# play-with-HOI-generation/HOIG

Hardware: AMD Instinct MI355X
Metric: HOGAN train images/sec at 256x256 (higher is better)
Workload: dtype f16x3 fwd (both operands split hi+lo on fp16, 3 MFMAs per product) / bf16x2 bwd (dy split hi+lo, weights and x single bf16, 2 MFMAs per product), f32 accumulate; 1 GPU; 256x256 HO3Dv3-shaped synthetic, batch 8 per GPU, G+D full step (generator_spade_attn, VGG19 surrogate weights); global_batch=8, parallelism=dp1

## Files before the change

hoig_amd/csrc/common.h:

```cpp
#pragma once
#include <hip/hip_runtime.h>
#include <stdint.h>
#include <atomic>
#include "hoig_kernels.h"

typedef float f32x16 __attribute__((ext_vector_type(16)));
typedef float f32x4 __attribute__((ext_vector_type(4)));
typedef short bf16x8 __attribute__((ext_vector_type(8)));

#define HOIG_LAUNCH_CHECK()                                   \
    do {                                                      \
        hipError_t e__ = hipGetLastError();                   \
        if (e__ != hipSuccess) return HOIG_ELAUNCH;           \
    } while (0)

struct hoig_once {
    std::atomic<unsigned long long> mask{0};
    static int dev() {
        int d = 0;
        (void)hipGetDevice(&d);
        return d & 63;
    }
    bool done() const { return (mask.load(std::memory_order_acquire) >> dev()) & 1ull; }
    void set() { mask.fetch_or(1ull << dev(), std::memory_order_release); }
};

static inline int64_t hoig_cdiv(int64_t a, int64_t b) { return (a + b - 1) / b; }

int hoig_conv_small_fwd(const hoig_conv_desc *d, const float *x, const float *w, const float *bias, float *y, hipStream_t st);
int hoig_conv_small_fwd_acts(const hoig_conv_desc *d, const float *x, const float *w, const float *bias, float *y,
                             unsigned long long acts, hipStream_t st);
int hoig_conv_small_ci_fwd(const hoig_conv_desc *d, const float *x, const float *w, const float *bias, float *y, hipStream_t st);
int hoig_conv_small_dgrad(const hoig_conv_desc *d, const float *dy, const float *w, float *dx, hipStream_t st);
int hoig_conv_small_wgrad(const hoig_conv_desc *d, const float *x, const float *dy, float *dw, hipStream_t st);
int hoig_conv_dot_fwd(const hoig_conv_desc *d, const float *x, const float *w, const float *bias, float *y, hipStream_t st);
int hoig_conv_head7_m16(const hoig_conv_desc *d, const float *x, const float *w, const float *bias, float *y, unsigned long long acts,
                        hipStream_t st);
int hoig_conv_thin_fwd(const hoig_conv_desc *d, const float *x, const float *w, const float *bias, float *y, hipStream_t st,
                       double *stats = nullptr);
int hoig_conv_thin_dgrad(const hoig_conv_desc *d, const float *dy, const float *w, float *dx, int accumulate, hipStream_t st);
int hoig_conv_thin_wgrad(const hoig_conv_desc *d, const float *x, const float *dy, float *dw, hipStream_t st);
bool hoig_conv_thin_wgrad_applies(const hoig_conv_desc *d);
int hoig_conv_thin_out(const hoig_conv_desc *d, const float *x, const float *w, const float *bias, float *y, unsigned long long acts,
                       int dgrad, hipStream_t st);
int hoig_conv_bf16_wgrad(const hoig_conv_desc *d, const float *x, const float *dy, float *dw, float *dbias, hipStream_t st);
bool hoig_conv_bf16_wgrad_fuses_bias(const hoig_conv_desc *d);
namespace hoig_detail { void *stream_scratch(hipStream_t st, size_t bytes); }

static inline int hoig_stream_grid(int64_t work_items, int block) {
    int64_t g = hoig_cdiv(work_items, block);
    if (g > 2048) g = 2048;
    if (g < 1) g = 1;
    return (int)g;
}

__device__ __forceinline__ float hoig_act(float v, int act, float slope) {
    switch (act) {
        case HOIG_ACT_RELU: return v > 0.f ? v : 0.f;
        case HOIG_ACT_LRELU: return v > 0.f ? v : v * slope;
        case HOIG_ACT_TANH: return tanhf(v);
        case HOIG_ACT_SIGMOID: return 1.f / (1.f + expf(-v));
        default: return v;
    }
}

__device__ __forceinline__ float fast_act(float v, float nslope, bool special, int act, float slope) {
    if (special) return hoig_act(v, act, slope);
    return v > 0.f ? v : fmaf(v, nslope, 0.f);
}

__device__ __forceinline__ float hoig_act_grad_from_y(float y, int act, float slope) {
    switch (act) {
        case HOIG_ACT_RELU: return y > 0.f ? 1.f : 0.f;
        case HOIG_ACT_LRELU: return y > 0.f ? 1.f : slope;
        case HOIG_ACT_TANH: return 1.f - y * y;
        case HOIG_ACT_SIGMOID: return y * (1.f - y);
        default: return 1.f;
    }
}

__device__ __forceinline__ void hoig_stats_add(double *stats, int b, int N, int mom, int n, float v) {
    atomicAdd(stats + ((size_t)b * 2 + mom) * N + n, (double)v);
}

__device__ __forceinline__ int hoig_xcd_remap(int bid, int nblk) {
    const int q = nblk >> 3, r = nblk & 7, xcd = bid & 7, idx = bid >> 3;
    const int base = xcd < r ? xcd * (q + 1) : r * (q + 1) + (xcd - r) * q;
    return base + idx;
}

__device__ __forceinline__ float hoig_wave_sum(float v) {
#pragma unroll
    for (int o = 32; o > 0; o >>= 1) v += __shfl_xor(v, o, 64);
    return v;
}

__device__ __forceinline__ unsigned short hoig_f2bf(float f) {
    unsigned int u = __float_as_uint(f);
    u += 0x7FFFu + ((u >> 16) & 1u);
    return (unsigned short)(u >> 16);
}
__device__ __forceinline__ float hoig_bf2f(unsigned short h) { return __uint_as_float(((unsigned int)h) << 16); }
```

hoig_amd/csrc/conv_thin.hip:

```cpp
#include "common.h"
#include <map>
#include <mutex>

namespace {

typedef _Float16 f16x8 __attribute__((ext_vector_type(8)));
typedef short s16x4 __attribute__((ext_vector_type(4)));

constexpr int TH = 4, TW = 32, NTHR = 256;

struct ThinArgs {
    const float *T;
    const float *D;
    const float *bias;
    float *Out;
    float *Ws;
    int Bn, H, W, F, CD, KS, pad;
    int flip;
    int sj, st, sf;
    int act;
    float slope;
    int accumulate;
    float wscale;
    int K, KP, N, NP;
    int tiles_x, tiles_y, ntiles, strip;
    int HR, CW;
    double *stats;
};

template <bool FP16>
__device__ __forceinline__ void split16(float x, unsigned short &hi, unsigned short &lo) {
    if (FP16) {
        const _Float16 h = (_Float16)x;
        const _Float16 l = (_Float16)(x - (float)h);
        hi = __builtin_bit_cast(unsigned short, h);
        lo = __builtin_bit_cast(unsigned short, l);
    } else {
        const __bf16 h = (__bf16)x;
        hi = __builtin_bit_cast(unsigned short, h);
        const __bf16 l = (__bf16)(x - hoig_bf2f(hi));
        lo = __builtin_bit_cast(unsigned short, l);
    }
}

template <bool FP16>
__device__ __forceinline__ f32x16 mfma16(const bf16x8 a, const bf16x8 b, const f32x16 c) {
    if (FP16) return __builtin_amdgcn_mfma_f32_32x32x16_f16(__builtin_bit_cast(f16x8, a), __builtin_bit_cast(f16x8, b), c, 0, 0, 0);
    return __builtin_amdgcn_mfma_f32_32x32x16_bf16(a, b, c, 0, 0, 0);
}

constexpr int HMAX = 12;
struct HaloRegs {
    float v[HMAX];
};
struct HaloMap {
    int lds[HMAX];
    int rc[HMAX];
    int rounds;
};
__device__ __forceinline__ void halo_map(const ThinArgs &p, HaloMap &m) {
    const int wr = TW + p.KS - 1;
    const int row_elems = wr * p.F;
    const int total = p.HR * row_elems;
    m.rounds = (total + NTHR - 1) / NTHR;
#pragma unroll
    for (int it = 0; it < HMAX; ++it) {
        const int i = threadIdx.x + it * NTHR;
        m.lds[it] = -1;
        m.rc[it] = 0;
        if (i < total) {
            const int hy = i / row_elems, e = i - hy * row_elems;
            const int hx = e / p.F, f = e - hx * p.F;
            m.lds[it] = (f * p.HR + hy) * p.CW + hx;
            m.rc[it] = hy | (hx << 8) | (f << 16);
        }
    }
}
__device__ __forceinline__ void halo_load(const ThinArgs &p, const HaloMap &m, int b, int y0, int x0, HaloRegs &h) {
    const float *img = p.T + (size_t)b * p.H * p.W * p.F;
#pragma unroll
    for (int it = 0; it < HMAX; ++it) {
        h.v[it] = 0.f;
        if (it < m.rounds && m.lds[it] >= 0) {
            const int gy = y0 - p.pad + (m.rc[it] & 255), gx = x0 - p.pad + ((m.rc[it] >> 8) & 255);
            if (gy >= 0 && gy < p.H && gx >= 0 && gx < p.W) h.v[it] = img[((size_t)gy * p.W + gx) * p.F + (m.rc[it] >> 16)];
        }
    }
}
template <bool FP16, int NT>
__device__ __forceinline__ void halo_store(const ThinArgs &p, const HaloMap &m, const HaloRegs &h, unsigned short *Tl) {
    const int plane = p.F * p.HR * p.CW;
#pragma unroll
    for (int it = 0; it < HMAX; ++it)
        if (it < m.rounds && m.lds[it] >= 0) {
            unsigned short hi, lo;
            split16<FP16>(h.v[it], hi, lo);
            Tl[m.lds[it]] = hi;
            if (NT == 2) Tl[plane + m.lds[it]] = lo;
        }
}

__device__ __forceinline__ void tile_coords(const ThinArgs &p, int t, int &b, int &y0, int &x0) {
    const int tx = t % p.tiles_x;
    t /= p.tiles_x;
    const int ty = t % p.tiles_y;
    b = t / p.tiles_y;
    y0 = ty * TH;
    x0 = tx * TW;
}

template <bool FP16, int NT, int NW>
__global__ __launch_bounds__(NTHR) void thin_gemm_kernel(const ThinArgs p) {
    extern __shared__ __attribute__((aligned(16))) unsigned char smem[];
    const int wstride = p.KP + 8;
    unsigned short *Wl = reinterpret_cast<unsigned short *>(smem);
    unsigned short *toff = Wl + NW * 64 * wstride;
    unsigned short *Tl = toff + p.KP;
    const int tid = threadIdx.x, lane = tid & 63, wave = tid >> 6;
    const int l31 = lane & 31, lh = lane >> 5;
    const int cbase = blockIdx.y * 64;
    const int KK = p.KS * p.KS;
    const int tplane = p.F * p.HR * p.CW;

    for (int i0 = tid; i0 < 64 * p.KP; i0 += 4 * NTHR) {
        float v[4];
        int dst[4];
#pragma unroll
        for (int u = 0; u < 4; ++u) {
            const int i = i0 + u * NTHR;
            v[u] = 0.f;
            dst[u] = -1;
            if (i < 64 * p.KP) {
                const int n = i / p.KP, k = i - n * p.KP;
                dst[u] = n * wstride + k;
                if (k < p.K) {
                    const int tap = k / p.F, f = k - tap * p.F;
                    const int tw = p.flip ? KK - 1 - tap : tap;
                    v[u] = p.D[(size_t)(cbase + n) * p.sj + (size_t)tw * p.st + (size_t)f * p.sf];
                }
            }
        }
#pragma unroll
        for (int u = 0; u < 4; ++u)
            if (dst[u] >= 0) {
                unsigned short hi, lo;
                split16<FP16>(v[u] * p.wscale, hi, lo);
                Wl[dst[u]] = hi;
                if (NW == 2) Wl[64 * wstride + dst[u]] = lo;
            }
    }
    for (int k = tid; k < p.KP; k += NTHR) {
        const int kc = k < p.K ? k : p.K - 1;
        const int tap = kc / p.F, f = kc - tap * p.F;
        const int r = tap / p.KS, s = tap - r * p.KS;
        toff[k] = (unsigned short)((f * p.HR + r) * p.CW + s);
    }

    const float nslope = p.act == HOIG_ACT_NONE ? 1.f : (p.act == HOIG_ACT_RELU ? 0.f : p.slope);
    const bool special = p.act == HOIG_ACT_TANH || p.act == HOIG_ACT_SIGMOID;
    const float inv = 1.f / p.wscale;
    float bias_r[2];
#pragma unroll
    for (int j = 0; j < 2; ++j) bias_r[j] = p.bias ? p.bias[cbase + j * 32 + l31] : 0.f;
    const int ksteps = p.KP >> 4;
    const int pix = wave * p.CW + l31;

    const int t_end = min(p.ntiles, (int)(blockIdx.x + 1) * p.strip);
    HaloRegs hreg;
    HaloMap hmap;
    halo_map(p, hmap);
    {
        int b, y0, x0;
        tile_coords(p, blockIdx.x * p.strip, b, y0, x0);
        halo_load(p, hmap, b, y0, x0, hreg);
    }
    float st1[2] = {0.f, 0.f}, st2[2] = {0.f, 0.f};
    int sb = -1;
    auto flush_stats = [&]() {
        if (sb >= 0) {
#pragma unroll
            for (int j = 0; j < 2; ++j) {
                const float s1 = st1[j] + __shfl_xor(st1[j], 32), s2 = st2[j] + __shfl_xor(st2[j], 32);
                if (lh == 0) {
                    hoig_stats_add(p.stats, sb, p.CD, 0, cbase + j * 32 + l31, s1);
                    hoig_stats_add(p.stats, sb, p.CD, 1, cbase + j * 32 + l31, s2);
                }
                st1[j] = st2[j] = 0.f;
            }
        }
    };
    for (int t = blockIdx.x * p.strip; t < t_end; ++t) {
        int b, y0, x0;
        tile_coords(p, t, b, y0, x0);
        if (p.stats && b != sb) {
            flush_stats();
            sb = b;
        }
        __syncthreads();
        halo_store<FP16, NT>(p, hmap, hreg, Tl);
        __syncthreads();
        if (t + 1 < t_end) {
            int b2, y2, x2;
            tile_coords(p, t + 1, b2, y2, x2);
            halo_load(p, hmap, b2, y2, x2, hreg);
        }
        f32x16 acc[2];
#pragma unroll
        for (int j = 0; j < 2; ++j)
#pragma unroll
            for (int r = 0; r < 16; ++r) acc[j][r] = 0.f;
#pragma unroll 1
        for (int kk = 0; kk < ksteps; ++kk) {
            const int k0 = kk * 16 + lh * 8;
            const bf16x8 offs = *reinterpret_cast<const bf16x8 *>(toff + k0);
            bf16x8 a0, a1;
#pragma unroll
            for (int e = 0; e < 8; ++e) {
                const int o = (int)(unsigned short)offs[e] + pix;
                a0[e] = (short)Tl[o];
                if (NT == 2) a1[e] = (short)Tl[tplane + o];
            }
#pragma unroll
            for (int j = 0; j < 2; ++j) {
                const unsigned short *wr = Wl + (j * 32 + l31) * wstride + k0;
                const bf16x8 w0 = *reinterpret_cast<const bf16x8 *>(wr);
                if (NT == 2) acc[j] = mfma16<FP16>(a1, w0, acc[j]);
                if (NW == 2) acc[j] = mfma16<FP16>(a0, *reinterpret_cast<const bf16x8 *>(wr + 64 * wstride), acc[j]);
                acc[j] = mfma16<FP16>(a0, w0, acc[j]);
            }
        }
        const int oy = y0 + wave;
#pragma unroll
        for (int r = 0; r < 16; ++r) {
            const int ox = x0 + (r & 3) + 8 * (r >> 2) + 4 * lh;
            float *dst = p.Out + (((size_t)b * p.H + oy) * p.W + ox) * p.CD + cbase + l31;
#pragma unroll
            for (int j = 0; j < 2; ++j) {
                float v = acc[j][r] * inv + bias_r[j];
                v = fast_act(v, nslope, special, p.act, p.slope);
                if (p.accumulate) v += dst[j * 32];
                dst[j * 32] = v;
                st1[j] += v;
                st2[j] += v * v;
            }
        }
    }
    if (p.stats) flush_stats();
}

constexpr int DROW = 192;

template <int NPW, int WN, int NT, int ND>
__global__ __launch_bounds__(NTHR) void thin_wgrad_kernel(const ThinArgs p) {
    constexpr int WK = 4 / WN, NPIX = TH * TW, KSTEPS = NPIX / 16;
    extern __shared__ __attribute__((aligned(16))) unsigned char smem[];
    unsigned char *Dl = smem;
    unsigned short *Tl = reinterpret_cast<unsigned short *>(smem + ND * NPIX * DROW);
    float *Gl = reinterpret_cast<float *>(smem);
    const int tid = threadIdx.x, lane = tid & 63, wave = tid >> 6;
    const int l31 = lane & 31, lh = lane >> 5;
    const int wn = wave % WN, wk = wave / WN;
    const int cbase = blockIdx.y * 64;
    const int KK = p.KS * p.KS;
    const int tplane = p.F * p.HR * p.CW;

    int noff[NPW];
    bool nval[NPW];
#pragma unroll
    for (int j = 0; j < NPW; ++j) {
        const int n = (wn * NPW + j) * 32 + l31;
        nval[j] = n < p.N;
        const int nc = nval[j] ? n : 0;
        const int tap = nc / p.F, f = nc - tap * p.F;
        const int tt = p.flip ? KK - 1 - tap : tap;
        const int r = tt / p.KS, s = tt - r * p.KS;
        noff[j] = (f * p.HR + r) * p.CW + s + lh * 8;
    }
    const int g = lane >> 4, q = (lane >> 2) & 3, pp = lane & 3;
    const int a_off = (8 * (g >> 1) + q) * DROW + (16 * (g & 1) + 4 * pp) * 2;

    f32x16 acc[2][NPW];
#pragma unroll
    for (int i = 0; i < 2; ++i)
#pragma unroll
        for (int j = 0; j < NPW; ++j)
#pragma unroll
            for (int r = 0; r < 16; ++r) acc[i][j][r] = 0.f;

    constexpr int DT = NPIX * 8 / NTHR;
    float4 dreg[DT][2];
    auto load_d = [&](int t) {
        int b, y0, x0;
        tile_coords(p, t, b, y0, x0);
#pragma unroll
        for (int i = 0; i < DT; ++i) {
            const int task = tid + i * NTHR, px = task >> 3, c8 = task & 7;
            const int yy = y0 + (px >> 5), xx = x0 + (px & 31);
            const float *src = p.D + (((size_t)b * p.H + yy) * p.W + xx) * p.CD + cbase + c8 * 8;
            dreg[i][0] = *reinterpret_cast<const float4 *>(src);
            dreg[i][1] = *reinterpret_cast<const float4 *>(src + 4);
        }
    };
    auto store_d = [&]() {
#pragma unroll
        for (int i = 0; i < DT; ++i) {
            const int task = tid + i * NTHR, px = task >> 3, c8 = task & 7;
            const float v[8] = {dreg[i][0].x, dreg[i][0].y, dreg[i][0].z, dreg[i][0].w,
                                dreg[i][1].x, dreg[i][1].y, dreg[i][1].z, dreg[i][1].w};
            bf16x8 hi, lo;
#pragma unroll
            for (int e = 0; e < 8; e += 2) {
                typedef float f2v __attribute__((ext_vector_type(2)));
                typedef __bf16 b2v __attribute__((ext_vector_type(2)));
                const f2v x2 = {v[e], v[e + 1]};
                const unsigned hp = __builtin_bit_cast(unsigned, __builtin_convertvector(x2, b2v));
                hi[e] = (short)(hp & 0xffffu);
                hi[e + 1] = (short)(hp >> 16);
                if (ND == 2) {
                    const f2v r2 = {v[e] - __uint_as_float(hp << 16), v[e + 1] - __uint_as_float(hp & 0xffff0000u)};
                    const unsigned lp = __builtin_bit_cast(unsigned, __builtin_convertvector(r2, b2v));
                    lo[e] = (short)(lp & 0xffffu);
                    lo[e + 1] = (short)(lp >> 16);
                }
            }
            *reinterpret_cast<bf16x8 *>(Dl + px * DROW + c8 * 16) = hi;
            if (ND == 2) *reinterpret_cast<bf16x8 *>(Dl + NPIX * DROW + px * DROW + c8 * 16) = lo;
        }
    };

    int t = blockIdx.x;
    HaloRegs hreg;
    HaloMap hmap;
    halo_map(p, hmap);
    if (t < p.ntiles) {
        int b, y0, x0;
        tile_coords(p, t, b, y0, x0);
        load_d(t);
        halo_load(p, hmap, b, y0, x0, hreg);
    }
    for (; t < p.ntiles; t += gridDim.x) {
        __syncthreads();
        store_d();
        halo_store<false, NT>(p, hmap, hreg, Tl);
        __syncthreads();
        if (t + (int)gridDim.x < p.ntiles) {
            int b, y0, x0;
            tile_coords(p, t + gridDim.x, b, y0, x0);
            load_d(t + gridDim.x);
            halo_load(p, hmap, b, y0, x0, hreg);
        }
#pragma unroll 1
        for (int ks = wk; ks < KSTEPS; ks += WK) {
            const int prow = ks >> 1, pcol = (ks & 1) * 16;
            bf16x8 a[2][ND];
#pragma unroll
            for (int i = 0; i < 2; ++i)
#pragma unroll
                for (int d = 0; d < ND; ++d) {
                    const unsigned char *src = Dl + d * NPIX * DROW + (prow * 32 + pcol) * DROW + a_off + i * 64;
                    const s16x4 v0 = __builtin_amdgcn_ds_read_tr16_b64_v4i16((__attribute__((address_space(3))) s16x4 *)(src));
                    const s16x4 v1 = __builtin_amdgcn_ds_read_tr16_b64_v4i16((__attribute__((address_space(3))) s16x4 *)(src + 4 * DROW));
                    a[i][d] = (bf16x8){v0[0], v0[1], v0[2], v0[3], v1[0], v1[1], v1[2], v1[3]};
                }
            const int base = prow * p.CW + pcol;
#pragma unroll
            for (int j = 0; j < NPW; ++j) {
                bf16x8 b0, b1;
#pragma unroll
                for (int e = 0; e < 8; ++e) {
                    const int o = base + noff[j] + e;
                    b0[e] = nval[j] ? (short)Tl[o] : (short)0;
                    if (NT == 2) b1[e] = nval[j] ? (short)Tl[tplane + o] : (short)0;
                }
#pragma unroll
                for (int i = 0; i < 2; ++i) {
                    if (ND == 2) acc[i][j] = mfma16<false>(a[i][1], b0, acc[i][j]);
                    if (NT == 2) acc[i][j] = mfma16<false>(a[i][0], b1, acc[i][j]);
                    acc[i][j] = mfma16<false>(a[i][0], b0, acc[i][j]);
                }
            }
        }
    }

    __syncthreads();
    for (int i = tid; i < 64 * p.NP; i += NTHR) Gl[i] = 0.f;
    __syncthreads();
#pragma unroll
    for (int i = 0; i < 2; ++i)
#pragma unroll
        for (int j = 0; j < NPW; ++j) {
            const int n = (wn * NPW + j) * 32 + l31;
            if (n < p.NP)
#pragma unroll
                for (int r = 0; r < 16; ++r) {
                    const int m = i * 32 + (r & 3) + 8 * (r >> 2) + 4 * lh;
                    if (WK > 1) atomicAdd(&Gl[m * p.NP + n], acc[i][j][r]);
                    else Gl[m * p.NP + n] = acc[i][j][r];
                }
        }
    __syncthreads();
    if (p.Ws) {
        float *dst = p.Ws + ((size_t)blockIdx.y * gridDim.x + blockIdx.x) * 64 * p.NP;
        for (int i = tid; i < 64 * p.NP; i += NTHR) dst[i] = Gl[i];
        return;
    }
    if (p.sj == 1) {
        for (int i = tid; i < 64 * p.N; i += NTHR) {
            const int n = i >> 6, m = i & 63;
            const int tap = n / p.F, f = n - tap * p.F;
            atomicAdd(p.Out + (size_t)f * p.sf + (size_t)tap * p.st + cbase + m, Gl[m * p.NP + n]);
        }
    } else {
        for (int i = tid; i < 64 * p.N; i += NTHR) {
            const int m = i / p.N, n = i - m * p.N;
            const int tap = n / p.F, f = n - tap * p.F;
            atomicAdd(p.Out + (size_t)(cbase + m) * p.sj + (size_t)tap * p.st + (size_t)f * p.sf, Gl[m * p.NP + n]);
        }
    }
}

__global__ __launch_bounds__(NTHR) void thin_reduce_kernel(const ThinArgs p, int nwg) {
    const int cbase = blockIdx.y * 64;
    const float *src = p.Ws + (size_t)blockIdx.y * nwg * 64 * p.NP;
    const int i = blockIdx.x * NTHR + threadIdx.x;
    if (i >= 64 * p.N) return;
    const int m = i / p.N, n = i - m * p.N;
    const int wper = (nwg + (int)gridDim.z - 1) / (int)gridDim.z;
    const int w0 = blockIdx.z * wper, w1 = min(nwg, w0 + wper);
    const size_t step = (size_t)64 * p.NP;
    const float *col = src + m * p.NP + n + (size_t)w0 * step;
    float v0 = 0.f, v1 = 0.f, v2 = 0.f, v3 = 0.f;
    int w = w0;
    for (; w + 3 < w1; w += 4, col += 4 * step) {
        v0 += col[0];
        v1 += col[step];
        v2 += col[2 * step];
        v3 += col[3 * step];
    }
    for (; w < w1; ++w, col += step) v0 += col[0];
    const float v = (v0 + v1) + (v2 + v3);
    const int tap = n / p.F, f = n - tap * p.F;
    atomicAdd(p.Out + (size_t)(cbase + m) * p.sj + (size_t)tap * p.st + (size_t)f * p.sf, v);
}

constexpr size_t WS_SLOT_BYTES = (size_t)16 << 20;
float *thin_workspace(hipStream_t st, size_t bytes) { return static_cast<float *>(hoig_detail::stream_scratch(st, bytes)); }

typedef float f32x4v __attribute__((ext_vector_type(4)));

struct ThinOutArgs {
    const float *D, *Wt, *bias;
    float *Out;
    int Bn, H, W, F, CD, KS, pad, flip;
    int sf, st, sj;
    unsigned long long acts;
    float slope, wscale;
    int tiles_x, tiles_y, ntiles, strip, HR, HWc;
};

template <bool FP16>
__device__ __forceinline__ f32x4v mfma16x16(const bf16x8 a, const bf16x8 b, const f32x4v c) {
    if (FP16) return __builtin_amdgcn_mfma_f32_16x16x32_f16(__builtin_bit_cast(f16x8, a), __builtin_bit_cast(f16x8, b), c, 0, 0, 0);
    return __builtin_amdgcn_mfma_f32_16x16x32_bf16(a, b, c, 0, 0, 0);
}

template <bool FP16, int ND, int NW>
__global__ __launch_bounds__(NTHR) void thin_out_kernel(const ThinOutArgs p) {
    constexpr int PROW = 80, WROW = 144;
    extern __shared__ __attribute__((aligned(16))) unsigned char smem[];
    const int KK = p.KS * p.KS, hpix = p.HR * p.HWc;
    unsigned char *Wl = smem;
    unsigned char *Dl = smem + (size_t)NW * (p.CD >> 6) * p.F * KK * WROW;
    const int tid = threadIdx.x, lane = tid & 63, wave = tid >> 6;
    const int l15 = lane & 15, kg = lane >> 4;
    const int wplane = p.F * KK * WROW;

    for (int i0 = tid; i0 < p.F * KK * p.CD; i0 += 4 * NTHR) {
        float v[4];
        int dst[4];
#pragma unroll
        for (int u = 0; u < 4; ++u) {
            const int i = i0 + u * NTHR;
            v[u] = 0.f;
            dst[u] = -1;
            if (i < p.F * KK * p.CD) {
                const int j = i % p.CD, ft = i / p.CD;
                const int tap = ft % KK, f = ft / KK;
                const int tw = p.flip ? KK - 1 - tap : tap;
                v[u] = p.Wt[(size_t)f * p.sf + (size_t)tw * p.st + (size_t)j * p.sj];
                dst[u] = ((j >> 6) * p.F * KK + f * KK + tap) * WROW + (j & 63) * 2;
            }
        }
#pragma unroll
        for (int u = 0; u < 4; ++u)
            if (dst[u] >= 0) {
                unsigned short hi, lo;
                split16<FP16>(v[u] * p.wscale, hi, lo);
                *reinterpret_cast<unsigned short *>(Wl + dst[u]) = hi;
                if (NW == 2) *reinterpret_cast<unsigned short *>(Wl + (size_t)(p.CD >> 6) * wplane + dst[u]) = lo;
            }
    }

    int apix[2];
#pragma unroll
    for (int i = 0; i < 2; ++i) {
        const int g = 2 * wave + i;
        apix[i] = ((g >> 1) * p.HWc + 16 * (g & 1) + l15) * PROW + kg * 16;
    }
    const bool nvalid = l15 < p.F;
    const int wrow0 = l15 * KK * WROW + kg * 16;
    const float inv = 1.f / p.wscale;
    const int act_n = (int)((p.acts >> (4 * l15)) & 15);
    const float bias_n = (p.bias && nvalid) ? p.bias[l15] : 0.f;

    constexpr int HT = 12;
    float4 hreg[HT];
    auto halo_load = [&](int t, int kh) {
        int b, y0, x0;
        const int tx = t % p.tiles_x, r1 = t / p.tiles_x;
        b = r1 / p.tiles_y;
        y0 = (r1 % p.tiles_y) * TH;
        x0 = tx * TW;
#pragma unroll
        for (int it = 0; it < HT; ++it) {
            const int i = tid + it * NTHR;
            hreg[it] = make_float4(0.f, 0.f, 0.f, 0.f);
            if (it * NTHR < hpix * 8 && i < hpix * 8) {
                const int px = i >> 3, c4 = i & 7;
                const int hy = px / p.HWc, hx = px - hy * p.HWc;
                const int gy = y0 - p.pad + hy, gx = x0 - p.pad + hx;
                if (gy >= 0 && gy < p.H && gx >= 0 && gx < p.W)
                    hreg[it] = *reinterpret_cast<const float4 *>(p.D + (((size_t)b * p.H + gy) * p.W + gx) * p.CD + kh * 32 + c4 * 4);
            }
        }
    };
    auto halo_store = [&]() {
#pragma unroll
        for (int it = 0; it < HT; ++it) {
            const int i = tid + it * NTHR;
            if (it * NTHR < hpix * 8 && i < hpix * 8) {
                const int px = i >> 3, c4 = i & 7;
                const float v[4] = {hreg[it].x, hreg[it].y, hreg[it].z, hreg[it].w};
                unsigned short h[4], l[4];
#pragma unroll
                for (int e = 0; e < 4; ++e) split16<FP16>(v[e], h[e], l[e]);
                *reinterpret_cast<uint2 *>(Dl + px * PROW + c4 * 8) = make_uint2(h[0] | ((unsigned)h[1] << 16), h[2] | ((unsigned)h[3] << 16));
                if (ND == 2)
                    *reinterpret_cast<uint2 *>(Dl + hpix * PROW + px * PROW + c4 * 8) =
                        make_uint2(l[0] | ((unsigned)l[1] << 16), l[2] | ((unsigned)l[3] << 16));
            }
        }
    };

    const int nkh = p.CD >> 5;
    const int t_begin = blockIdx.x * p.strip, t_end = min(p.ntiles, t_begin + p.strip);
    if (t_begin < t_end) halo_load(t_begin, 0);
    for (int t = t_begin; t < t_end; ++t) {
        f32x4v acc[2];
#pragma unroll
        for (int i = 0; i < 2; ++i) acc[i] = (f32x4v){0.f, 0.f, 0.f, 0.f};
        for (int kh = 0; kh < nkh; ++kh) {
            __syncthreads();
            halo_store();
            __syncthreads();
            if (kh + 1 < nkh) halo_load(t, kh + 1);
            else if (t + 1 < t_end) halo_load(t + 1, 0);
            const unsigned char *wbase = Wl + (size_t)(kh >> 1) * wplane + wrow0 + (kh & 1) * 64;
#pragma unroll 1
            for (int tap = 0; tap < KK; ++tap) {
                const int r = tap / p.KS, s_ = tap - r * p.KS;
                const int toff = (r * p.HWc + s_) * PROW;
                bf16x8 bh = {0, 0, 0, 0, 0, 0, 0, 0}, bl = bh;
                if (nvalid) {
                    bh = *reinterpret_cast<const bf16x8 *>(wbase + tap * WROW);
                    if (NW == 2) bl = *reinterpret_cast<const bf16x8 *>(wbase + (size_t)(p.CD >> 6) * wplane + tap * WROW);
                }
#pragma unroll
                for (int i = 0; i < 2; ++i) {
                    const unsigned char *ap = Dl + apix[i] + toff;
                    const bf16x8 ah = *reinterpret_cast<const bf16x8 *>(ap);
                    if (ND == 2) acc[i] = mfma16x16<FP16>(*reinterpret_cast<const bf16x8 *>(ap + hpix * PROW), bh, acc[i]);
                    if (NW == 2) acc[i] = mfma16x16<FP16>(ah, bl, acc[i]);
                    acc[i] = mfma16x16<FP16>(ah, bh, acc[i]);
                }
            }
        }
        if (nvalid) {
            const int tx = t % p.tiles_x, r1 = t / p.tiles_x;
            const int b = r1 / p.tiles_y, y0 = (r1 % p.tiles_y) * TH, x0 = tx * TW;
#pragma unroll
            for (int i = 0; i < 2; ++i) {
                const int g = 2 * wave + i;
                const int oy = y0 + (g >> 1), oxb = x0 + 16 * (g & 1) + 4 * kg;
#pragma unroll
                for (int e = 0; e < 4; ++e) {
                    const float v = acc[i][e] * inv + bias_n;
                    p.Out[(((size_t)b * p.H + oy) * p.W + oxb + e) * p.F + l15] = hoig_act(v, act_n, p.slope);
                }
            }
        }
    }
}

bool thin_geometry(const hoig_conv_desc *d) {
    return !d->transposed && d->stride == 1 && d->R == d->S && (d->R & 1) && d->R <= 7 && 2 * d->pad == d->R - 1 &&
           d->Ho == d->Hi && d->Wo == d->Wi && (d->Hi % TH) == 0 && (d->Wi % TW) == 0;
}

void fill_common(ThinArgs &a, const hoig_conv_desc *d, int F, int CD) {
    a.Bn = d->B; a.H = d->Hi; a.W = d->Wi; a.F = F; a.CD = CD; a.KS = d->R; a.pad = d->pad;
    a.K = d->R * d->S * F;
    a.KP = (a.K + 15) / 16 * 16;
    a.N = a.K;
    a.NP = (a.N + 31) / 32 * 32;
    a.tiles_x = d->Wi / TW; a.tiles_y = d->Hi / TH;
    a.ntiles = d->B * a.tiles_x * a.tiles_y;
    a.HR = TH + d->R - 1;
    a.CW = (TW + d->R - 1 + 8 + 1) & ~1;
    a.bias = nullptr; a.act = HOIG_ACT_NONE; a.slope = 0.f; a.accumulate = 0; a.wscale = 1.f; a.strip = 1; a.Ws = nullptr; a.stats = nullptr;
}

template <bool FP16>
int launch_gemm(const ThinArgs &a, int precision, hipStream_t st) {
    const int nt = precision == HOIG_PREC_BF16 ? 1 : 2, nw = precision == HOIG_PREC_BF16X3 ? 2 : 1;
    const size_t smem = (size_t)nw * 64 * (a.KP + 8) * 2 + (size_t)a.KP * 2 + (size_t)nt * a.F * a.HR * a.CW * 2;
    if (smem > 160 * 1024) return HOIG_EUNSUPPORTED;
    dim3 grid((unsigned)hoig_cdiv(a.ntiles, a.strip), a.CD / 64);
#define HOIG_THIN_GEMM(NT_, NW_)                                                                                         \
    do {                                                                                                                 \
        static hoig_once attr;                                                                                        \
        if (!attr.done()) {                                                                                                     \
            if (hipFuncSetAttribute(reinterpret_cast<const void *>(&thin_gemm_kernel<FP16, NT_, NW_>),                   \
                                    hipFuncAttributeMaxDynamicSharedMemorySize, 160 * 1024) != hipSuccess)               \
                return HOIG_ELAUNCH;                                                                                     \
            attr.set();                                                                                                 \
        }                                                                                                                \
        thin_gemm_kernel<FP16, NT_, NW_><<<grid, NTHR, smem, st>>>(a);                                                   \
    } while (0)
    if (nt == 2 && nw == 2) HOIG_THIN_GEMM(2, 2);
    else if (nt == 2) HOIG_THIN_GEMM(2, 1);
    else HOIG_THIN_GEMM(1, 1);
#undef HOIG_THIN_GEMM
    HOIG_LAUNCH_CHECK();
    return HOIG_OK;
}

template <int NPW, int WN>
int launch_wgrad_t(const ThinArgs &a, int nt, int nd, dim3 grid, size_t smem, hipStream_t st) {
#define HOIG_THIN_WG(NT_, ND_)                                                                                           \
    do {                                                                                                                 \
        static hoig_once attr;                                                                                        \
        if (!attr.done()) {                                                                                                     \
            if (hipFuncSetAttribute(reinterpret_cast<const void *>(&thin_wgrad_kernel<NPW, WN, NT_, ND_>),               \
                                    hipFuncAttributeMaxDynamicSharedMemorySize, 160 * 1024) != hipSuccess)               \
                return HOIG_ELAUNCH;                                                                                     \
            attr.set();                                                                                                 \
        }                                                                                                                \
        thin_wgrad_kernel<NPW, WN, NT_, ND_><<<grid, NTHR, smem, st>>>(a);                                               \
    } while (0)
    if (nt == 2 && nd == 2) HOIG_THIN_WG(2, 2);
    else if (nt == 2) HOIG_THIN_WG(2, 1);
    else if (nd == 2) HOIG_THIN_WG(1, 2);
    else HOIG_THIN_WG(1, 1);
#undef HOIG_THIN_WG
    HOIG_LAUNCH_CHECK();
    return HOIG_OK;
}

}

int hoig_conv_thin_fwd(const hoig_conv_desc *d, const float *x, const float *w, const float *bias, float *y, hipStream_t st, double *stats) {
    if (d->precision == HOIG_PREC_F32 || !thin_geometry(d) || d->Ci > (d->R <= 3 ? 12 : 8) || d->Ci < 1 || (d->Co % 64)) return HOIG_EUNSUPPORTED;
    ThinArgs a;
    fill_common(a, d, d->Ci, d->Co);
    a.T = x; a.D = w; a.bias = bias; a.Out = y; a.stats = stats;
    a.flip = 0;
    a.sj = d->R * d->S * d->Ci; a.st = d->Ci; a.sf = 1;
    a.act = d->act; a.slope = d->slope;
    a.wscale = 256.f;
    a.strip = a.ntiles >= 4096 ? 8 : (a.ntiles >= 1024 ? 4 : 1);
    return launch_gemm<true>(a, d->precision, st);
}

int hoig_conv_thin_dgrad(const hoig_conv_desc *d, const float *dy, const float *w, float *dx, int accumulate, hipStream_t st) {
    if (d->precision == HOIG_PREC_F32 || !thin_geometry(d) || d->Co > 8 || d->Co < 1 || (d->Ci % 64)) return HOIG_EUNSUPPORTED;
    ThinArgs a;
    fill_common(a, d, d->Co, d->Ci);
    a.T = dy; a.D = w; a.Out = dx;
    a.flip = 1;
    a.sj = 1; a.st = d->Ci; a.sf = d->R * d->S * d->Ci;
    a.accumulate = accumulate;
    a.strip = a.ntiles >= 4096 ? 8 : (a.ntiles >= 1024 ? 4 : 1);
    return launch_gemm<false>(a, d->precision, st);
}

bool hoig_conv_thin_wgrad_applies(const hoig_conv_desc *d) {
    if (d->precision == HOIG_PREC_F32 || !thin_geometry(d)) return false;
    return (d->Ci <= (d->R <= 3 ? 12 : 8) && (d->Co % 64) == 0) || (d->Co <= 8 && (d->Ci % 64) == 0);
}

int hoig_conv_thin_wgrad(const hoig_conv_desc *d, const float *x, const float *dy, float *dw, hipStream_t st) {
    if (d->precision == HOIG_PREC_F32 || !thin_geometry(d)) return HOIG_EUNSUPPORTED;
    const bool thin_in = d->Ci <= (d->R <= 3 ? 12 : 8) && (d->Co % 64) == 0, thin_out = d->Co <= 8 && (d->Ci % 64) == 0;
    if (!thin_in && !thin_out) return HOIG_EUNSUPPORTED;
    ThinArgs a;
    int nt, nd;
    if (thin_in) {
        fill_common(a, d, d->Ci, d->Co);
        a.T = x; a.D = dy; a.flip = 0;
        a.sj = d->R * d->S * d->Ci; a.st = d->Ci; a.sf = 1;
        nd = d->precision == HOIG_PREC_BF16 ? 1 : 2;
        nt = d->precision == HOIG_PREC_BF16X3 ? 2 : 1;
    } else {
        fill_common(a, d, d->Co, d->Ci);
        a.T = dy; a.D = x; a.flip = 1;
        a.sj = 1; a.st = d->Ci; a.sf = d->R * d->S * d->Ci;
        nt = d->precision == HOIG_PREC_BF16 ? 1 : 2;
        nd = d->precision == HOIG_PREC_BF16X3 ? 2 : 1;
    }
    a.Out = dw;
    const int nfr = a.NP / 32;
    if (nfr > 16) return HOIG_EUNSUPPORTED;
    size_t smem = (size_t)nd * TH * TW * DROW + (size_t)nt * a.F * a.HR * a.CW * 2;
    const size_t gsm = (size_t)64 * a.NP * 4;
    if (gsm > smem) smem = gsm;
    if (smem > 160 * 1024) return HOIG_EUNSUPPORTED;
    int nwg = 512;
    if (smem > 80 * 1024 || a.N >= 128) nwg = 256;
    if (nwg > a.ntiles) nwg = a.ntiles;
    const int groups = a.CD / 64;
    while (nwg > 64 && (size_t)nwg * groups * 64 * a.NP * 4 > WS_SLOT_BYTES) nwg >>= 1;
    dim3 grid(nwg, groups);
    a.Ws = nwg > 8 ? thin_workspace(st, (size_t)nwg * groups * 64 * a.NP * 4) : nullptr;
    int rc;
    if (nfr == 1) rc = launch_wgrad_t<1, 1>(a, nt, nd, grid, smem, st);
    else if (nfr == 2) rc = launch_wgrad_t<2, 1>(a, nt, nd, grid, smem, st);
    else if (nfr <= 4) rc = launch_wgrad_t<2, 2>(a, nt, nd, grid, smem, st);
    else if (nfr <= 8) rc = launch_wgrad_t<2, 4>(a, nt, nd, grid, smem, st);
    else rc = launch_wgrad_t<4, 4>(a, nt, nd, grid, smem, st);
    if (rc != HOIG_OK || !a.Ws) return rc;
    thin_reduce_kernel<<<dim3((unsigned)hoig_cdiv(64 * a.N, NTHR), groups, (unsigned)hoig_cdiv(nwg, 32)), NTHR, 0, st>>>(a, nwg);
    HOIG_LAUNCH_CHECK();
    return HOIG_OK;
}

int hoig_conv_thin_out(const hoig_conv_desc *d, const float *x, const float *w, const float *bias, float *y,
                       unsigned long long acts, int dgrad, hipStream_t st) {
    if (d->precision == HOIG_PREC_F32 || !thin_geometry(d)) return HOIG_EUNSUPPORTED;
    const int F = dgrad ? d->Ci : d->Co, CD = dgrad ? d->Co : d->Ci;
    if (F < 1 || F > 16 || (CD % 64)) return HOIG_EUNSUPPORTED;
    if (d->R > 3) return HOIG_EUNSUPPORTED;
    ThinOutArgs a;
    a.D = x; a.Wt = w; a.bias = bias; a.Out = y;
    a.Bn = d->B; a.H = d->Hi; a.W = d->Wi; a.F = F; a.CD = CD; a.KS = d->R; a.pad = d->pad;
    const int KK = d->R * d->S;
    if (!dgrad) { a.flip = 0; a.sf = KK * CD; a.st = CD; a.sj = 1; a.wscale = 256.f; }
    else { a.flip = 1; a.sf = 1; a.st = F; a.sj = KK * F; a.wscale = 1.f; }
    a.acts = acts; a.slope = d->slope;
    a.tiles_x = d->Wi / TW; a.tiles_y = d->Hi / TH; a.ntiles = d->B * a.tiles_x * a.tiles_y;
    a.strip = a.ntiles >= 2048 ? 8 : (a.ntiles >= 512 ? 2 : 1);
    a.HR = TH + d->R - 1; a.HWc = TW + d->R - 1;
    if (a.HR * a.HWc * 8 > 12 * NTHR) return HOIG_EUNSUPPORTED;
    const int nd = d->precision == HOIG_PREC_BF16 ? 1 : 2, nw = d->precision == HOIG_PREC_BF16X3 ? 2 : 1;
    const size_t smem = (size_t)nw * (CD / 64) * F * KK * 144 + (size_t)nd * a.HR * a.HWc * 80;
    if (smem > 160 * 1024) return HOIG_EUNSUPPORTED;
    const unsigned grid = (unsigned)hoig_cdiv(a.ntiles, a.strip);
#define HOIG_THIN_OUT(FP16_, ND_, NW_)                                                                                   \
    do {                                                                                                                 \
        static hoig_once attr;                                                                                        \
        if (!attr.done()) {                                                                                                     \
            if (hipFuncSetAttribute(reinterpret_cast<const void *>(&thin_out_kernel<FP16_, ND_, NW_>),                   \
                                    hipFuncAttributeMaxDynamicSharedMemorySize, 160 * 1024) != hipSuccess)               \
                return HOIG_ELAUNCH;                                                                                     \
            attr.set();                                                                                                 \
        }                                                                                                                \
        thin_out_kernel<FP16_, ND_, NW_><<<grid, NTHR, smem, st>>>(a);                                                   \
    } while (0)
    if (!dgrad) {
        if (nd == 2 && nw == 2) HOIG_THIN_OUT(true, 2, 2);
        else if (nd == 2) HOIG_THIN_OUT(true, 2, 1);
        else HOIG_THIN_OUT(true, 1, 1);
    } else {
        if (nd == 2 && nw == 2) HOIG_THIN_OUT(false, 2, 2);
        else if (nd == 2) HOIG_THIN_OUT(false, 2, 1);
        else HOIG_THIN_OUT(false, 1, 1);
    }
#undef HOIG_THIN_OUT
    HOIG_LAUNCH_CHECK();
    return HOIG_OK;
}
```

hoig_amd/csrc/tuning.h:

```cpp
#pragma once
enum HoigTuning { HOIG_TUNE_IGEMM16 = 0, HOIG_TUNE_S2_16, HOIG_TUNE_FLAT5, HOIG_TUNE_WFLAT5, HOIG_TUNE_HEAD16, HOIG_TUNE_D_EARLY, HOIG_TUNE_SPLIT_GRADS, HOIG_TUNE_PAIR, HOIG_TUNE_WDMA16, HOIG_TUNE_S2_PIPE, HOIG_TUNE_NORM_IN, HOIG_TUNE_WINO8, HOIG_TUNE_HALO5, HOIG_TUNE_COUNT };
int hoig_tuning(int id);
```

hoig_amd/csrc/tuning.hip:

```cpp
#include <cstring>
#include "hoig_kernels.h"
#include "tuning.h"

namespace {
struct Entry {
    const char *key;
    int value;
};
Entry g_table[HOIG_TUNE_COUNT] = {
    {"igemm16", 1},
    {"s2_16", 1},
    {"flat5", 2},
    {"wflat5", 1},
    {"head16", 1},
    {"d_early", 1},
    {"split_grads", 1},
    {"pair", 2},
    {"wdma16", 2},
    {"s2_pipe", 1},
    {"norm_in", 1},
    {"wino8", 0},
    {"halo5", 1},
};
}

int hoig_tuning(int id) { return (id >= 0 && id < HOIG_TUNE_COUNT) ? g_table[id].value : 0; }

extern "C" int hoig_set_tuning(const char *key, int value) {
    if (!key) return -1;
    for (int i = 0; i < HOIG_TUNE_COUNT; ++i)
        if (strcmp(g_table[i].key, key) == 0) {
            const int prev = g_table[i].value;
            if (value >= 0) g_table[i].value = value;
            return prev;
        }
    return -1;
}
```

Before: 130.9 images/s.

## Add 16x16x32 MFMA thin-channel 7x7 conv kernel for fwd and dgrad

```diff
diff --git a/hoig_amd/csrc/common.h b/hoig_amd/csrc/common.h
--- a/hoig_amd/csrc/common.h
+++ b/hoig_amd/csrc/common.h
@@ -43,6 +43,8 @@
 bool hoig_conv_thin_wgrad_applies(const hoig_conv_desc *d);
 int hoig_conv_thin_out(const hoig_conv_desc *d, const float *x, const float *w, const float *bias, float *y, unsigned long long acts,
                        int dgrad, hipStream_t st);
+int hoig_conv_thin16_fwd(const hoig_conv_desc *d, const float *x, const float *w, const float *bias, float *y, hipStream_t st, double *stats);
+int hoig_conv_thin16_dgrad(const hoig_conv_desc *d, const float *dy, const float *w, float *dx, int accumulate, hipStream_t st);
 int hoig_conv_bf16_wgrad(const hoig_conv_desc *d, const float *x, const float *dy, float *dw, float *dbias, hipStream_t st);
 bool hoig_conv_bf16_wgrad_fuses_bias(const hoig_conv_desc *d);
 namespace hoig_detail { void *stream_scratch(hipStream_t st, size_t bytes); }
diff --git a/hoig_amd/csrc/conv_thin.hip b/hoig_amd/csrc/conv_thin.hip
--- a/hoig_amd/csrc/conv_thin.hip
+++ b/hoig_amd/csrc/conv_thin.hip
@@ -1,4 +1,5 @@
 #include "common.h"
+#include "tuning.h"
 #include <map>
 #include <mutex>
 
@@ -670,6 +671,10 @@
 }
 
 int hoig_conv_thin_fwd(const hoig_conv_desc *d, const float *x, const float *w, const float *bias, float *y, hipStream_t st, double *stats) {
+    if (hoig_tuning(HOIG_TUNE_THIN16) >= 1) {
+        const int rc = hoig_conv_thin16_fwd(d, x, w, bias, y, st, stats);
+        if (rc != HOIG_EUNSUPPORTED) return rc;
+    }
     if (d->precision == HOIG_PREC_F32 || !thin_geometry(d) || d->Ci > (d->R <= 3 ? 12 : 8) || d->Ci < 1 || (d->Co % 64)) return HOIG_EUNSUPPORTED;
     ThinArgs a;
     fill_common(a, d, d->Ci, d->Co);
@@ -683,6 +688,10 @@
 }
 
 int hoig_conv_thin_dgrad(const hoig_conv_desc *d, const float *dy, const float *w, float *dx, int accumulate, hipStream_t st) {
+    if (hoig_tuning(HOIG_TUNE_THIN16) >= 1) {
+        const int rc = hoig_conv_thin16_dgrad(d, dy, w, dx, accumulate, st);
+        if (rc != HOIG_EUNSUPPORTED) return rc;
+    }
     if (d->precision == HOIG_PREC_F32 || !thin_geometry(d) || d->Co > 8 || d->Co < 1 || (d->Ci % 64)) return HOIG_EUNSUPPORTED;
     ThinArgs a;
     fill_common(a, d, d->Co, d->Ci);
diff --git a/hoig_amd/csrc/conv_thin16.hip b/hoig_amd/csrc/conv_thin16.hip
--- /dev/null
+++ b/hoig_amd/csrc/conv_thin16.hip
@@ -0,0 +1,334 @@
+#include "common.h"
+#include "tuning.h"
+
+namespace {
+
+typedef _Float16 f16x8 __attribute__((ext_vector_type(8)));
+
+constexpr int TH = 4, TW = 32, NTHR = 256;
+constexpr int CWP = 40;
+
+struct Thin16Args {
+    const float *T;
+    const float *Wt;
+    const float *bias;
+    float *Out;
+    double *stats;
+    int Bn, H, W, F, CD, pad;
+    int flip;
+    int sj, st, sf;
+    int act;
+    float slope;
+    int accumulate;
+    float wscale;
+    int tiles_x, tiles_y, ntiles, strip;
+};
+
+template <bool FP16>
+__device__ __forceinline__ void split16(float x, unsigned short &hi, unsigned short &lo) {
+    if (FP16) {
+        const _Float16 h = (_Float16)x;
+        const _Float16 l = (_Float16)(x - (float)h);
+        hi = __builtin_bit_cast(unsigned short, h);
+        lo = __builtin_bit_cast(unsigned short, l);
+    } else {
+        const __bf16 h = (__bf16)x;
+        hi = __builtin_bit_cast(unsigned short, h);
+        const __bf16 l = (__bf16)(x - hoig_bf2f(hi));
+        lo = __builtin_bit_cast(unsigned short, l);
+    }
+}
+
+template <bool FP16>
+__device__ __forceinline__ f32x4 mfma16x16(const bf16x8 a, const bf16x8 b, const f32x4 c) {
+    if (FP16) return __builtin_amdgcn_mfma_f32_16x16x32_f16(__builtin_bit_cast(f16x8, a), __builtin_bit_cast(f16x8, b), c, 0, 0, 0);
+    return __builtin_amdgcn_mfma_f32_16x16x32_bf16(a, b, c, 0, 0, 0);
+}
+
+template <int FP>
+__device__ __forceinline__ bf16x8 window_read(const unsigned short *src) {
+    if (FP == 8) return *reinterpret_cast<const bf16x8 *>(src);
+    const uint2 a = *reinterpret_cast<const uint2 *>(src), b = *reinterpret_cast<const uint2 *>(src + 4);
+    const uint4 v = make_uint4(a.x, a.y, b.x, b.y);
+    return __builtin_bit_cast(bf16x8, v);
+}
+
+__device__ __forceinline__ void tile_coords(const Thin16Args &p, int t, int &b, int &y0, int &x0) {
+    const int tx = t % p.tiles_x;
+    t /= p.tiles_x;
+    const int ty = t % p.tiles_y;
+    b = t / p.tiles_y;
+    y0 = ty * TH;
+    x0 = tx * TW;
+}
+
+template <bool FP16, int NT, int NW, int KS, int FP, int MT>
+__global__ __launch_bounds__(NTHR, MT == 1 ? 2 : 1) void thin16_gemm_kernel(const Thin16Args p) {
+    constexpr int KW = (KS * FP + 31) / 32;
+    constexpr int HR = TH + KS - 1, HPIX = HR * CWP;
+    constexpr int ROUNDS = (HPIX + NTHR - 1) / NTHR;
+    constexpr int KK = KS * KS;
+    constexpr int CD = 64 * MT, OROW = CD + 4;
+    extern __shared__ __attribute__((aligned(16))) unsigned char smem[];
+    unsigned short *Tl = reinterpret_cast<unsigned short *>(smem);
+    float *Ol = reinterpret_cast<float *>(smem + NT * HPIX * FP * 2);
+    const int tid = threadIdx.x, lane = tid & 63, wave = tid >> 6;
+    const int l15 = lane & 15, lg = lane >> 4;
+
+    bf16x8 wh[MT][KS][KW], wl[MT][KS][KW];
+#pragma unroll
+    for (int m = 0; m < MT; ++m) {
+        const size_t jrow = (size_t)((m * 4 + wave) * 16 + l15) * p.sj;
+#pragma unroll
+        for (int r = 0; r < KS; ++r)
+#pragma unroll
+            for (int ks = 0; ks < KW; ++ks) {
+                float v[8];
+#pragma unroll
+                for (int e = 0; e < 8; ++e) {
+                    const int k = ks * 32 + lg * 8 + e, s = k / FP, f = k % FP;
+                    const int tap = r * KS + s, tw = p.flip ? KK - 1 - tap : tap;
+                    v[e] = (s < KS && f < p.F) ? p.Wt[jrow + (size_t)tw * p.st + (size_t)f * p.sf] : 0.f;
+                }
+#pragma unroll
+                for (int e = 0; e < 8; ++e) {
+                    unsigned short hi, lo;
+                    split16<FP16>(v[e] * p.wscale, hi, lo);
+                    wh[m][r][ks][e] = (short)hi;
+                    if (NW == 2) wl[m][r][ks][e] = (short)lo;
+                }
+            }
+    }
+
+    const float nslope = p.act == HOIG_ACT_NONE ? 1.f : (p.act == HOIG_ACT_RELU ? 0.f : p.slope);
+    const bool special = p.act == HOIG_ACT_TANH || p.act == HOIG_ACT_SIGMOID;
+    const float inv = 1.f / p.wscale;
+    float bias_r[MT][4];
+#pragma unroll
+    for (int m = 0; m < MT; ++m)
+#pragma unroll
+        for (int e = 0; e < 4; ++e) bias_r[m][e] = p.bias ? p.bias[(m * 4 + wave) * 16 + lg * 4 + e] : 0.f;
+
+    float hreg[ROUNDS][FP];
+    auto halo_load = [&](int t) {
+        int b, y0, x0;
+        tile_coords(p, t, b, y0, x0);
+        const float *img = p.T + (size_t)b * p.H * p.W * p.F;
+#pragma unroll
+        for (int it = 0; it < ROUNDS; ++it) {
+            const int i = tid + it * NTHR, hy = i / CWP, hx = i - hy * CWP;
+            const int gy = y0 - p.pad + hy, gx = x0 - p.pad + hx;
+            const bool in = i < HPIX && hx < TW + KS - 1 && gy >= 0 && gy < p.H && gx >= 0 && gx < p.W;
+            const float *src = img + ((size_t)(in ? gy : 0) * p.W + (in ? gx : 0)) * p.F;
+#pragma unroll
+            for (int f = 0; f < FP; ++f) hreg[it][f] = (in && f < p.F) ? src[f] : 0.f;
+        }
+    };
+    auto halo_store = [&]() {
+#pragma unroll
+        for (int it = 0; it < ROUNDS; ++it) {
+            const int i = tid + it * NTHR;
+            if (i < HPIX) {
+                unsigned hp[FP / 2], lp[FP / 2];
+#pragma unroll
+                for (int f = 0; f < FP; f += 2) {
+                    unsigned short h0, l0, h1, l1;
+                    split16<FP16>(hreg[it][f], h0, l0);
+                    split16<FP16>(hreg[it][f + 1], h1, l1);
+                    hp[f / 2] = h0 | ((unsigned)h1 << 16);
+                    lp[f / 2] = l0 | ((unsigned)l1 << 16);
+                }
+                if (FP == 8) {
+                    *reinterpret_cast<uint4 *>(Tl + i * FP) = make_uint4(hp[0], hp[1], hp[FP / 2 - 2], hp[FP / 2 - 1]);
+                    if (NT == 2) *reinterpret_cast<uint4 *>(Tl + HPIX * FP + i * FP) = make_uint4(lp[0], lp[1], lp[FP / 2 - 2], lp[FP / 2 - 1]);
+                } else {
+                    *reinterpret_cast<uint2 *>(Tl + i * FP) = make_uint2(hp[0], hp[1]);
+                    if (NT == 2) *reinterpret_cast<uint2 *>(Tl + HPIX * FP + i * FP) = make_uint2(lp[0], lp[1]);
+                }
+            }
+        }
+    };
+
+    float st1[MT][4], st2[MT][4];
+#pragma unroll
+    for (int m = 0; m < MT; ++m)
+#pragma unroll
+        for (int e = 0; e < 4; ++e) st1[m][e] = st2[m][e] = 0.f;
+    int sb = -1;
+    auto flush_stats = [&]() {
+        if (sb >= 0) {
+#pragma unroll
+            for (int m = 0; m < MT; ++m)
+#pragma unroll
+                for (int e = 0; e < 4; ++e) {
+                    float s1 = st1[m][e], s2 = st2[m][e];
+#pragma unroll
+                    for (int o = 1; o < 16; o <<= 1) {
+                        s1 += __shfl_xor(s1, o);
+                        s2 += __shfl_xor(s2, o);
+                    }
+                    if (l15 == 0) {
+                        hoig_stats_add(p.stats, sb, p.CD, 0, (m * 4 + wave) * 16 + lg * 4 + e, s1);
+                        hoig_stats_add(p.stats, sb, p.CD, 1, (m * 4 + wave) * 16 + lg * 4 + e, s2);
+                    }
+                    st1[m][e] = st2[m][e] = 0.f;
+                }
+        }
+    };
+
+    const int t_begin = blockIdx.x * p.strip, t_end = min(p.ntiles, t_begin + p.strip);
+    if (t_begin < t_end) halo_load(t_begin);
+    for (int t = t_begin; t < t_end; ++t) {
+        int b, y0, x0;
+        tile_coords(p, t, b, y0, x0);
+        if (p.stats && b != sb) {
+            flush_stats();
+            sb = b;
+        }
+        __syncthreads();
+        halo_store();
+        __syncthreads();
+        if (t + 1 < t_end) halo_load(t + 1);
+#pragma unroll 1
+        for (int row = 0; row < TH; ++row) {
+            f32x4 acc[MT][2][2], acx[MT][2];
+#pragma unroll
+            for (int m = 0; m < MT; ++m)
+#pragma unroll
+                for (int c = 0; c < 2; ++c) acc[m][c][0] = acc[m][c][1] = acx[m][c] = (f32x4){0.f, 0.f, 0.f, 0.f};
+            const unsigned short *win = Tl + (row * CWP + l15) * FP + lg * 8;
+#pragma unroll
+            for (int r = 0; r < KS; ++r)
+#pragma unroll
+                for (int ks = 0; ks < KW; ++ks) {
+                    bf16x8 bh[2], bl[2];
+#pragma unroll
+                    for (int c = 0; c < 2; ++c) {
+                        const unsigned short *src = win + (r * CWP + c * 16) * FP + ks * 32;
+                        bh[c] = window_read<FP>(src);
+                        if (NT == 2) bl[c] = window_read<FP>(src + HPIX * FP);
+                    }
+#pragma unroll
+                    for (int m = 0; m < MT; ++m)
+#pragma unroll
+                        for (int c = 0; c < 2; ++c) {
+                            if (NT == 2) acx[m][c] = mfma16x16<FP16>(wh[m][r][ks], bl[c], acx[m][c]);
+                            if (NW == 2) acx[m][c] = mfma16x16<FP16>(wl[m][r][ks], bh[c], acx[m][c]);
+                            acc[m][c][r & 1] = mfma16x16<FP16>(wh[m][r][ks], bh[c], acc[m][c][r & 1]);
+                        }
+                }
+            const int oy = y0 + row;
+#pragma unroll
+            for (int c = 0; c < 2; ++c) {
+                const int ox = x0 + c * 16 + l15;
+                const bool inside = oy < p.H && ox < p.W;
+#pragma unroll
+                for (int m = 0; m < MT; ++m) {
+                    float v[4];
+#pragma unroll
+                    for (int e = 0; e < 4; ++e) {
+                        const float main = acc[m][c][0][e] + acc[m][c][1][e];
+                        v[e] = (NT == 2 ? main + acx[m][c][e] : main) * inv + bias_r[m][e];
+                        v[e] = fast_act(v[e], nslope, special, p.act, p.slope);
+                    }
+                    if (p.accumulate && inside) {
+                        const float4 o = *reinterpret_cast<const float4 *>(p.Out + (((size_t)b * p.H + oy) * p.W + ox) * CD + (m * 4 + wave) * 16 + lg * 4);
+                        v[0] += o.x; v[1] += o.y; v[2] += o.z; v[3] += o.w;
+                    }
+                    *reinterpret_cast<float4 *>(Ol + (row * TW + c * 16 + l15) * OROW + (m * 4 + wave) * 16 + lg * 4) = make_float4(v[0], v[1], v[2], v[3]);
+                    if (inside) {
+#pragma unroll
+                        for (int e = 0; e < 4; ++e) {
+                            st1[m][e] += v[e];
+                            st2[m][e] += v[e] * v[e];
+                        }
+                    }
+                }
+            }
+        }
+        __syncthreads();
+#pragma unroll
+        for (int it = 0; it < TH * TW * CD / 4 / NTHR; ++it) {
+            const int i = tid + it * NTHR, px = i / (CD / 4), c4 = i - px * (CD / 4);
+            const int oy = y0 + px / TW, ox = x0 + px % TW;
+            if (oy < p.H && ox < p.W)
+                *reinterpret_cast<float4 *>(p.Out + (((size_t)b * p.H + oy) * p.W + ox) * CD + c4 * 4) =
+                    *reinterpret_cast<const float4 *>(Ol + px * OROW + c4 * 4);
+        }
+    }
+    if (p.stats) flush_stats();
+}
+
+template <bool FP16, int KS, int FP, int MT>
+int launch_prec(const Thin16Args &a, int precision, hipStream_t st) {
+    const int nt = precision == HOIG_PREC_BF16 ? 1 : 2, nw = precision == HOIG_PREC_BF16X3 ? 2 : 1;
+    const unsigned grid = (unsigned)hoig_cdiv(a.ntiles, a.strip);
+    const size_t smem = (size_t)nt * (TH + KS - 1) * CWP * FP * 2 + (size_t)TH * TW * (64 * MT + 4) * 4;
+#define HOIG_THIN16_GO(NT_, NW_)                                                                                         \
+    do {                                                                                                                 \
+        static hoig_once attr;                                                                                           \
+        if (!attr.done()) {                                                                                              \
+            if (hipFuncSetAttribute(reinterpret_cast<const void *>(&thin16_gemm_kernel<FP16, NT_, NW_, KS, FP, MT>),     \
+                                    hipFuncAttributeMaxDynamicSharedMemorySize, 96 * 1024) != hipSuccess)                \
+                return HOIG_ELAUNCH;                                                                                     \
+            attr.set();                                                                                                  \
+        }                                                                                                                \
+        thin16_gemm_kernel<FP16, NT_, NW_, KS, FP, MT><<<grid, NTHR, smem, st>>>(a);                                     \
+    } while (0)
+    if (nt == 2 && nw == 2) HOIG_THIN16_GO(2, 2);
+    else if (nt == 2) HOIG_THIN16_GO(2, 1);
+    else HOIG_THIN16_GO(1, 1);
+#undef HOIG_THIN16_GO
+    HOIG_LAUNCH_CHECK();
+    return HOIG_OK;
+}
+
+template <bool FP16>
+int launch_thin16(Thin16Args &a, int KS, int precision, hipStream_t st) {
+    a.tiles_x = (int)hoig_cdiv(a.W, TW);
+    a.tiles_y = (int)hoig_cdiv(a.H, TH);
+    a.ntiles = a.Bn * a.tiles_x * a.tiles_y;
+    a.strip = (int)hoig_cdiv(a.ntiles, 512);
+    const int fp = a.F <= 4 ? 4 : 8, mt = a.CD / 64;
+#define HOIG_THIN16(KS_, FP_)                                                                     \
+    if (KS == KS_ && fp == FP_)                                                                   \
+        return mt == 1 ? launch_prec<FP16, KS_, FP_, 1>(a, precision, st) : launch_prec<FP16, KS_, FP_, 2>(a, precision, st)
+    HOIG_THIN16(7, 8);
+    HOIG_THIN16(7, 4);
+#undef HOIG_THIN16
+    return HOIG_EUNSUPPORTED;
+}
+
+bool thin16_takes(const hoig_conv_desc *d, int F, int CD) {
+    if (d->precision == HOIG_PREC_F32 || d->transposed || d->stride != 1 || d->R != 7 || d->S != 7 || d->pad != 3 ||
+        d->Ho != d->Hi || d->Wo != d->Wi)
+        return false;
+    if (CD != 64 && CD != 128) return false;
+    return F >= 2 && F <= 8;
+}
+
+}
+
+int hoig_conv_thin16_fwd(const hoig_conv_desc *d, const float *x, const float *w, const float *bias, float *y, hipStream_t st, double *stats) {
+    if (!thin16_takes(d, d->Ci, d->Co)) return HOIG_EUNSUPPORTED;
+    Thin16Args a;
+    a.T = x; a.Wt = w; a.bias = bias; a.Out = y; a.stats = stats;
+    a.Bn = d->B; a.H = d->Hi; a.W = d->Wi; a.F = d->Ci; a.CD = d->Co; a.pad = d->pad;
+    a.flip = 0;
+    a.sj = d->R * d->S * d->Ci; a.st = d->Ci; a.sf = 1;
+    a.act = d->act; a.slope = d->slope; a.accumulate = 0;
+    a.wscale = 256.f;
+    return launch_thin16<true>(a, d->R, d->precision, st);
+}
+
+int hoig_conv_thin16_dgrad(const hoig_conv_desc *d, const float *dy, const float *w, float *dx, int accumulate, hipStream_t st) {
+    if (!thin16_takes(d, d->Co, d->Ci)) return HOIG_EUNSUPPORTED;
+    Thin16Args a;
+    a.T = dy; a.Wt = w; a.bias = nullptr; a.Out = dx; a.stats = nullptr;
+    a.Bn = d->B; a.H = d->Hi; a.W = d->Wi; a.F = d->Co; a.CD = d->Ci; a.pad = d->pad;
+    a.flip = 1;
+    a.sj = 1; a.st = d->Ci; a.sf = d->R * d->S * d->Ci;
+    a.act = HOIG_ACT_NONE; a.slope = 0.f; a.accumulate = accumulate;
+    a.wscale = 1.f;
+    return launch_thin16<false>(a, d->R, d->precision, st);
+}
diff --git a/hoig_amd/csrc/tuning.h b/hoig_amd/csrc/tuning.h
--- a/hoig_amd/csrc/tuning.h
+++ b/hoig_amd/csrc/tuning.h
@@ -1,3 +1,3 @@
 #pragma once
-enum HoigTuning { HOIG_TUNE_IGEMM16 = 0, HOIG_TUNE_S2_16, HOIG_TUNE_FLAT5, HOIG_TUNE_WFLAT5, HOIG_TUNE_HEAD16, HOIG_TUNE_D_EARLY, HOIG_TUNE_SPLIT_GRADS, HOIG_TUNE_PAIR, HOIG_TUNE_WDMA16, HOIG_TUNE_S2_PIPE, HOIG_TUNE_NORM_IN, HOIG_TUNE_WINO8, HOIG_TUNE_HALO5, HOIG_TUNE_COUNT };
+enum HoigTuning { HOIG_TUNE_IGEMM16 = 0, HOIG_TUNE_S2_16, HOIG_TUNE_FLAT5, HOIG_TUNE_WFLAT5, HOIG_TUNE_HEAD16, HOIG_TUNE_D_EARLY, HOIG_TUNE_SPLIT_GRADS, HOIG_TUNE_PAIR, HOIG_TUNE_WDMA16, HOIG_TUNE_S2_PIPE, HOIG_TUNE_NORM_IN, HOIG_TUNE_WINO8, HOIG_TUNE_HALO5, HOIG_TUNE_THIN16, HOIG_TUNE_COUNT };
 int hoig_tuning(int id);
diff --git a/hoig_amd/csrc/tuning.hip b/hoig_amd/csrc/tuning.hip
--- a/hoig_amd/csrc/tuning.hip
+++ b/hoig_amd/csrc/tuning.hip
@@ -21,6 +21,7 @@
     {"norm_in", 1},
     {"wino8", 0},
     {"halo5", 1},
+    {"thin16", 1},
 };
 }
 
```

New measurement: 131.8 images/s, median of 6. About the same (+0.7%).
